# alshai/Big-BWT

Measured on NVIDIA B200. Metric: pfp_parse_throughput, higher is better.
Workload: dtype u8/u32/u64 integer

## Files before the change

### big-bwt_b200/csrc/pfp_phrase.cu

```cuda
#include "pfp_common.cuh"
#include "pfp_stages.cuh"
#include "pfp_fp.cuh"
#include <stdlib.h>

__device__ __forceinline__ void load_chunk(const TextView &tv, i64 s0, u64 len, u64 o, bool special,
                                           u32 x[4]) {
    const u32 nbv = (u32)((len - o) < 16 ? (len - o) : 16);
    if (!special) {
        const i64 loc = s0 + (i64)o - tv.pos0;
        const u8 *p = tv.T + loc;
        const u32 bs = (u32)((uintptr_t)p & 3);
        const u32 *p4 = reinterpret_cast<const u32 *>(p - bs);
        u32 W[5];
        if ((u64)loc + 20 <= tv.n_buf) {
#pragma unroll
            for (int j = 0; j < 5; j++) W[j] = __ldg(p4 + j);
        } else {
            const u32 need = bs + nbv;
#pragma unroll
            for (int j = 0; j < 5; j++) W[j] = (4u * j < need) ? __ldg(p4 + j) : 0u;
        }
#pragma unroll
        for (int j = 0; j < 4; j++) x[j] = __funnelshift_r(W[j], W[j + 1], 8 * bs);
    } else {
// ... 293 lines not shown
        const u32 slot = __shfl_sync(0xffffffffu, res, leader) & ~UID_CREATOR;
        const u32 lchk = __shfl_sync(0xffffffffu, chk, leader);
        if (j < P) {
            if (chk != lchk) atomicOr((unsigned long long *)&flags[0], PFP_ERRBIT_COLLISION);
            __stcs(uid + j, lead ? res : slot);
            if (weight) {
                const u32 c = weight[j];
                const u32 old = atomicAdd(&tab[slot].val, c);
                if (old + c < old) atomicOr((unsigned long long *)&flags[0], PFP_ERRBIT_LIMIT);
            }
        }
    }
}

constexpr int TC_T = 256;
constexpr int TC_I = 4;
constexpr int TC_TILE = TC_T * TC_I;

__device__ __forceinline__ void load_uids(const u32 *__restrict__ uid, u64 n, u64 j, u32 v[TC_I]) {
    if (j + TC_I <= n) {
        const uint4 a = __ldcs(reinterpret_cast<const uint4 *>(uid + j));
        v[0] = a.x; v[1] = a.y; v[2] = a.z; v[3] = a.w;
    } else {
#pragma unroll
        for (int i = 0; i < TC_I; i++) v[i] = j + i < n ? uid[j + i] : 0u;
    }
}

__global__ void __launch_bounds__(TC_T) table_creators_k(const u32 *__restrict__ uid, u64 n,
                                                         u32 *__restrict__ tile_count) {
    __shared__ u32 sm[9];
    u32 v[TC_I];
    load_uids(uid, n, (u64)blockIdx.x * TC_TILE + (u64)threadIdx.x * TC_I, v);
    u32 c = 0;
#pragma unroll
    for (int i = 0; i < TC_I; i++) c += v[i] >> 31;
    u32 total;
    block_excl_scan_256(c, &total, sm);
    if (threadIdx.x == 0) tile_count[blockIdx.x] = total;
}

__global__ void __launch_bounds__(TC_T, 6) table_compact_k(u32 *__restrict__ uid, u64 n,
                                                        const u32 *__restrict__ tile_base,
                                                        const DictSlot *__restrict__ tab,
                                                        const u32 *__restrict__ len_in,
                                                        const u64 *__restrict__ ends, i64 first_start, u32 w,
                                                        u32 *__restrict__ slot_of_word,
                                                        u32 *__restrict__ rep, u32 *__restrict__ count,
                                                        u32 *__restrict__ ulen, u32 *__restrict__ uwords,
                                                        i64 *__restrict__ ustart ,
                                                        u64 *__restrict__ flags) {
    __shared__ u32 sm[9];
    __shared__ u32 s_max;
    __shared__ unsigned long long s_sum;
    if (threadIdx.x == 0) { s_max = 0; s_sum = 0; }
    const u64 j0 = (u64)blockIdx.x * TC_TILE + (u64)threadIdx.x * TC_I;
    u32 v[TC_I];
    load_uids(uid, n, j0, v);
    u32 c = 0;
#pragma unroll
    for (int i = 0; i < TC_I; i++) c += v[i] >> 31;
    u32 cnt[TC_I], len[TC_I];
    i64 st[TC_I];
#pragma unroll
    for (int i = 0; i < TC_I; i++) {
        const u64 j = j0 + i;
        const bool cr = (v[i] & UID_CREATOR) != 0;
        cnt[i] = cr ? tab[v[i] & ~UID_CREATOR].val : 0u;
        if (len_in) {
            len[i] = cr ? len_in[j] : 0u;
            st[i] = 0;
        } else {
            st[i] = cr ? (j ? (i64)ends[j - 1] - (i64)w + 1 : first_start) : 0;
            len[i] = cr ? (u32)((i64)ends[j] - st[i] + 1) : 0u;
        }
    }
    u32 total;
    u32 u = block_excl_scan_256(c, &total, sm) + tile_base[blockIdx.x];
    u32 mx = 0;
    u64 sum = 0;
#pragma unroll
    for (int i = 0; i < TC_I; i++) {
        if (!(v[i] & UID_CREATOR)) continue;
        slot_of_word[u] = v[i] & ~UID_CREATOR;
        uid[j0 + i] = u | UID_CREATOR;
        rep[u] = (u32)(j0 + i); count[u] = cnt[i]; ulen[u] = len[i]; uwords[u] = (len[i] + 7) >> 3;
        if (ustart) ustart[u] = st[i];
        mx = max(mx, len[i]);
        sum += len[i];
        u++;
    }
    mx = __reduce_max_sync(0xffffffffu, mx);
#pragma unroll
    for (int o = 16; o > 0; o >>= 1) sum += __shfl_xor_sync(0xffffffffu, sum, o);
    if ((threadIdx.x & 31) == 0 && sum) { atomicMax(&s_max, mx); atomicAdd(&s_sum, (unsigned long long)sum); }
    __syncthreads();
    if (threadIdx.x == 0 && s_sum) {
        atomicMax((unsigned long long *)&flags[2], (unsigned long long)s_max);
        atomicAdd((unsigned long long *)&flags[3], s_sum);
    }
}

__global__ void word_of_slot_k(const u32 *__restrict__ slot_of_word, u64 d, const u64 *__restrict__ d_ptr,
                               u32 *__restrict__ word_of_slot) {
    const u64 u = (u64)blockIdx.x * blockDim.x + threadIdx.x;
    if (u < (d_ptr ? *d_ptr : d)) word_of_slot[slot_of_word[u]] = (u32)u;
}

__device__ __forceinline__ u32 word_of(u32 v, const u32 *__restrict__ word_of_slot) {
    return (v & UID_CREATOR) ? v & ~UID_CREATOR : word_of_slot[v];
}

__global__ void uid_words_k(u32 *__restrict__ uid, u64 n, const u32 *__restrict__ word_of_slot) {
    const u64 q = (u64)blockIdx.x * blockDim.x + threadIdx.x;
    const u64 j = 4 * q;
    if (j + 4 <= n) {
        uint4 v = __ldcs(reinterpret_cast<const uint4 *>(uid) + q);
        v.x = word_of(v.x, word_of_slot); v.y = word_of(v.y, word_of_slot);
        v.z = word_of(v.z, word_of_slot); v.w = word_of(v.w, word_of_slot);
        __stcs(reinterpret_cast<uint4 *>(uid) + q, v);
    } else {
        for (u64 i = j; i < n; i++) uid[i] = word_of(uid[i], word_of_slot);
    }
}

static int uid_words(pfpb200_ctx *ctx, DictArrays *D, u64 n, u64 d_max, const u64 *d_ptr) {
    if (n && d_max) {
        u32 *word_of_slot = nullptr;
        PFP_TRY(pfp_alloc_t(ctx, &word_of_slot, D->slots));
        word_of_slot_k<<<pfp_blocks(d_max, 256), 256, 0, ctx->stream>>>(D->slot_of_word, d_max, d_ptr, word_of_slot);
        PFP_LAUNCHED(ctx);
        uid_words_k<<<pfp_blocks((n + 3) / 4, 256), 256, 0, ctx->stream>>>(D->uid, n, word_of_slot);
        PFP_LAUNCHED(ctx);
        PFP_TRY(pfp_free_now(ctx, word_of_slot));
    }
    PFP_TRY(pfp_free_now(ctx, D->slot_of_word));
    D->slot_of_word = nullptr;
    return PFPB200_OK;
}

int pfp_uid_words(pfpb200_ctx *ctx, DictArrays *D, u64 n) {
    return D->slot_of_word ? uid_words(ctx, D, n, D->d, nullptr) : PFPB200_OK;
}

static int table_words(pfpb200_ctx *ctx, const PhraseFp *rec, u64 n, DictSlot *tab, u64 cap,
                       const u32 *weight, const u32 *len_in, const u64 *ends, i64 first_start, u32 w,
                       u32 *uid, const DictArrays &D) {
    table_init_k<<<pfp_blocks(cap, 256), 256, 0, ctx->stream>>>(tab, cap);
    PFP_LAUNCHED(ctx);
    PFP_CUDA(ctx, cudaMemsetAsync(&ctx->d_flags[1], 0, 3 * sizeof(u64), ctx->stream));
    if (n == 0) return PFPB200_OK;
    int per_sm = 0;
    PFP_CUDA(ctx, cudaOccupancyMaxActiveBlocksPerMultiprocessor(&per_sm, table_insert_k, TI_T, 0));
    const u64 want = (n + TI_T - 1) / TI_T;
    const u64 resident = (u64)ctx->sm_count * (per_sm > 0 ? per_sm : 1);
    table_insert_k<<<(u32)(want < resident ? want : resident), TI_T, 0, ctx->stream>>>(
        rec, n, tab, cap, weight, ctx->weak_fp, uid, ctx->d_flags);
    PFP_LAUNCHED(ctx);
    const u32 nt = pfp_blocks(n, TC_TILE);
    u32 *tile = nullptr;
    PFP_TRY(pfp_alloc_t(ctx, &tile, nt));
    table_creators_k<<<nt, TC_T, 0, ctx->stream>>>(uid, n, tile);
    PFP_LAUNCHED(ctx);
    PFP_TRY(pfp_exclusive_scan_u32(ctx, tile, tile, nt, reinterpret_cast<u32 *>(&ctx->d_flags[1])));
    table_compact_k<<<nt, TC_T, 0, ctx->stream>>>(uid, n, tile, tab, len_in, ends, first_start, w, D.slot_of_word,
                                                  D.rep, D.count, D.ulen, D.uwords, D.ustart, ctx->d_flags);
    PFP_LAUNCHED(ctx);
    PFP_TRY(pfp_free_now(ctx, tile));
    return PFPB200_OK;
}

__device__ __forceinline__ u64 phrase_word8(const TextView &tv, i64 s0, u64 len, u64 k, bool special) {
    const u64 o = 8 * k;
    const u32 nbv = (u32)((len - o) < 8 ? (len - o) : 8);
    u64 v = 0;
    if (!special) {
        const u8 *p = tv.T + (s0 + (i64)o - tv.pos0);
        const u32 bs = (u32)((uintptr_t)p & 7);
        const u64 *p8 = reinterpret_cast<const u64 *>(p - bs);
        const u64 lo = __ldg(p8);
        if (bs) {
            const u64 hi = (bs + nbv > 8) ? __ldg(p8 + 1) : 0ull;
            v = (lo >> (8 * bs)) | (hi << (64 - 8 * bs));
        } else v = lo;
    } else {
        for (u32 b = 0; b < nbv; b++) v |= (u64)tv_byte(tv, s0 + (i64)o + b) << (8 * b);
    }
    if (nbv < 8) v &= (1ull << (8 * nbv)) - 1ull;
    return v;
}

__global__ void __launch_bounds__(PH_T) pool_copy_span_k(TextView tv, const i64 *__restrict__ ustart,
                                                         const u32 *__restrict__ ulen,
                                                         const u64 *__restrict__ uoff, u64 d,
                                                         u64 *__restrict__ pool) {
    const u32 lane = threadIdx.x & 31;
    for (u64 u0 = ((u64)blockIdx.x * PH_WARPS + (threadIdx.x >> 5)) * 32; u0 < d; u0 += (u64)gridDim.x * PH_WARPS * 32) {
        const u64 u = u0 + lane;
        const bool have = u < d;
        const i64 s0 = have ? ustart[u] : 0;
        const u32 len = have ? ulen[u] : 0u;
        const u64 off = have ? uoff[u] : 0ull;
        const u64 base = __shfl_sync(0xffffffffu, off, 0);
        const u32 nw = (len + 7) >> 3;
        u32 rel = have ? (u32)(off - base) : 0xFFFFFFFFu;
        const u32 endrel = have ? rel + nw : 0u;
        u32 total = endrel;
#pragma unroll
        for (int o = 16; o > 0; o >>= 1) total = max(total, __shfl_xor_sync(0xffffffffu, total, o));
        const bool special = have && (s0 < 0 || s0 + (i64)len > tv.n_global);
        for (u32 k0 = 0; k0 < total; k0 += 32) {
            const u32 k = k0 + lane;
            u32 j = 0;
#pragma unroll
            for (int step = 16; step > 0; step >>= 1) {
                const u32 t = __shfl_sync(0xffffffffu, rel, (j + step) & 31);
                if (j + step < 32 && t <= k) j += step;
            }
            const u32 rj = __shfl_sync(0xffffffffu, rel, j);
            const u32 lj = __shfl_sync(0xffffffffu, len, j);
            const i64 sj = __shfl_sync(0xffffffffu, s0, j);
            const int spj = __shfl_sync(0xffffffffu, (int)special, j);
            if (k < total) pool[base + k] = phrase_word8(tv, sj, lj, k - rj, spj != 0);
        }
    }
}

__global__ void __launch_bounds__(PH_T) verify_phrases_k(TextView tv, const u64 *__restrict__ ends,
                                                         i64 first_start, u32 w, u64 P,
                                                         const u32 *__restrict__ uid,
                                                         const u32 *__restrict__ ulen,
                                                         const u64 *__restrict__ uoff,
                                                         const u64 *__restrict__ pool,
                                                         u64 *__restrict__ flags) {
    const u32 lane = threadIdx.x & 31;
    for (u64 j = (u64)blockIdx.x * PH_WARPS + (threadIdx.x >> 5); j < P; j += (u64)gridDim.x * PH_WARPS) {
        const i64 e = (i64)ends[j];
        const i64 s0 = (j == 0) ? first_start : (i64)ends[j - 1] - (i64)w + 1;
        const u64 len = (u64)(e - s0 + 1);
        const u32 u = uid[j];
        bool bad = len != (u64)ulen[u];
        if (!bad) {
            const bool special = (s0 < 0) || (e >= tv.n_global);
            const u64 *src = pool + uoff[u];
            const u64 nw = (len + 7) >> 3;
            for (u64 k = lane; k < nw; k += 32) bad |= phrase_word8(tv, s0, len, k, special) != src[k];
        }
        if (__any_sync(0xffffffffu, bad) && lane == 0)
            atomicOr((unsigned long long *)&flags[0], PFP_ERRBIT_COLLISION);
    }
}

__global__ void __launch_bounds__(PH_T) verify_entries_k(u64 n, const u32 *__restrict__ uid_of_entry,
                                                         const u32 *__restrict__ rep,
                                                         const u32 *__restrict__ len_in,
                                                         const u64 *__restrict__ in_off,
                                                         const u64 *__restrict__ pool,
                                                         u64 *__restrict__ flags) {
    const u32 lane = threadIdx.x & 31;
    for (u64 i = (u64)blockIdx.x * PH_WARPS + (threadIdx.x >> 5); i < n; i += (u64)gridDim.x * PH_WARPS) {
        const u32 r = rep[uid_of_entry[i]];
        if (r == (u32)i) continue;
        bool bad = len_in[i] != len_in[r];
        if (!bad) {
            const u64 *a = pool + in_off[i], *b = pool + in_off[r];
            const u64 nw = ((u64)len_in[i] + 7) >> 3;
            for (u64 k = lane; k < nw; k += 32) bad |= a[k] != b[k];
        }
        if (__any_sync(0xffffffffu, bad) && lane == 0)
            atomicOr((unsigned long long *)&flags[0], PFP_ERRBIT_COLLISION);
    }
}

int pfp_hash_list(pfpb200_ctx *ctx, const TextView &tv, const PhraseArrays &ph, i64 first_start, u32 w,
                  const u32 *long_list, const u32 *long_count, u64 max_count) {
    u64 want = (max_count + PH_WARPS - 1) / PH_WARPS;
// ... 8 lines not shown
}

int pfp_records_range(pfpb200_ctx *ctx, const TextView &tv, const PhraseArrays &ph, u64 j0, u64 P, u32 w) {
    if (j0 >= P) return PFPB200_OK;
    phrase_records_k<<<pfp_blocks(P - j0, 256), 256, 0, ctx->stream>>>(tv, ph.ends, j0, P, w, ph.last, ph.sai);
    PFP_LAUNCHED(ctx);
    return PFPB200_OK;
}

int pfp_hash_stage(pfpb200_ctx *ctx, const TextView &tv, const PhraseArrays &ph, u64 P,
                   i64 first_start, u32 w) {
    u32 *long_list = nullptr, *long_count = nullptr;
    const u64 cap = P + 8;
    PFP_TRY(pfp_alloc_t(ctx, &long_list, (size_t)cap));
    PFP_TRY(pfp_alloc_t(ctx, &long_count, 1));
    PFP_CUDA(ctx, cudaMemsetAsync(long_count, 0, sizeof(u32), ctx->stream));
    phrase_records_k<<<pfp_blocks(P, 256), 256, 0, ctx->stream>>>(tv, ph.ends, 0, P, w, ph.last, ph.sai);
    PFP_LAUNCHED(ctx);
    u64 want = (P + PH_PER_BLOCK - 1) / PH_PER_BLOCK;
    u64 maxb = (u64)ctx->sm_count * 32;
    u32 nb = (u32)(want < maxb ? want : maxb);
    if (nb == 0) nb = 1;
    phrase_hash_k<<<nb, PH_T, 0, ctx->stream>>>(tv, ph, P, first_start, w, ctx->d_keys, long_list, long_count,
                                                (u32)cap, ctx->d_flags);
    PFP_LAUNCHED(ctx);
    PFP_TRY(pfp_hash_list(ctx, tv, ph, first_start, w, long_list, long_count, cap));
    PFP_TRY(pfp_free_now(ctx, long_list));
    PFP_TRY(pfp_free_now(ctx, long_count));
    return PFPB200_OK;
}

int pfp_dedup_stage(pfpb200_ctx *ctx, const PhraseArrays &ph, u64 P, i64 first_start, u32 w, DictArrays *D) {
    if (P >= 0x7FFFFFFEull) return pfp_fail(ctx, PFPB200_E_LIMIT, "more than 2^31-2 phrases in one shard");
    DictSlot *tab = nullptr;
    u64 cap = 0, d = 0;
    PFP_TRY(pfp_alloc_t(ctx, &D->uid, P));
    for (int attempt = 0;; attempt++) {
        double want = (double)P * 1.5;
        if (attempt == 0 && ctx->dedup_ratio > 0.0) {
            double guess = ctx->dedup_ratio * (double)P * 2.0;
            if (guess < want) want = guess;
        }
        cap = (u64)want + 1024;
        if (cap >= 0x7FFFFFFFull) cap = 0x7FFFFFFEull;
        const u64 wcap = cap < P ? cap : P;
        PFP_TRY(pfp_alloc_t(ctx, &tab, cap));
        PFP_TRY(pfp_alloc_t(ctx, &D->slot_of_word, wcap));
        PFP_TRY(pfp_alloc_t(ctx, &D->rep, wcap));
        PFP_TRY(pfp_alloc_t(ctx, &D->count, wcap));
        PFP_TRY(pfp_alloc_t(ctx, &D->ulen, wcap));
        PFP_TRY(pfp_alloc_t(ctx, &D->uwords, wcap));
        PFP_TRY(pfp_alloc_t(ctx, &D->ustart, wcap));
        PFP_TRY(table_words(ctx, ph.rec, P, tab, cap, nullptr, nullptr, ph.ends, first_start, w, D->uid, *D));
        PFP_CUDA(ctx, cudaMemcpyAsync(ctx->h_flags, ctx->d_flags, 4 * sizeof(u64), cudaMemcpyDeviceToHost,
                                      ctx->stream));
        PFP_CUDA(ctx, cudaStreamSynchronize(ctx->stream));
        if (ctx->h_flags[0] & PFP_ERRBIT_LIMIT)
            return pfp_fail(ctx, PFPB200_E_LIMIT, "a phrase is longer than 2^32-1 bytes");
        d = ctx->h_flags[1];
        const bool full = (ctx->h_flags[0] & PFP_ERRBIT_TABLE_FULL) != 0 || (double)d > 0.85 * (double)cap;
        if (!full) break;
        if (attempt > 0) return pfp_fail(ctx, PFPB200_E_INTERNAL, "dictionary table overflow");
        void *fr[] = {tab, D->slot_of_word, D->rep, D->count, D->ulen, D->uwords, D->ustart};
        for (void *q : fr) PFP_TRY(pfp_free_now(ctx, q));
        ctx->dedup_ratio = 0.0;
        const u64 keep = ctx->h_flags[0] & ~(PFP_ERRBIT_TABLE_FULL | PFP_ERRBIT_COLLISION);
        PFP_CUDA(ctx, cudaMemcpyAsync(&ctx->d_flags[0], &keep, sizeof(u64), cudaMemcpyHostToDevice, ctx->stream));
        PFP_CUDA(ctx, cudaStreamSynchronize(ctx->stream));
    }
    D->slots = cap;
    ctx->dedup_ratio = (double)d / (double)P;
    if (d > 0x7FFFFFFEull)
        return pfp_fail(ctx, PFPB200_E_LIMIT, "%llu distinct words exceed the limit 2^31-2",
                        (unsigned long long)d);
    D->d = d;
    D->max_len = (u32)ctx->h_flags[2];
    D->sum_len = ctx->h_flags[3];
    PFP_TRY(pfp_free_now(ctx, tab));
    return PFPB200_OK;
}

int pfp_pool_stage(pfpb200_ctx *ctx, const TextView &tv, DictArrays *D) {
    u64 d = D->d;
    PFP_TRY(pfp_alloc_t(ctx, &D->uoff, d));
    PFP_TRY(pfp_exclusive_scan_u32_u64(ctx, D->uwords, D->uoff, d, &ctx->d_flags[1]));
    PFP_CUDA(ctx, cudaMemcpyAsync(ctx->h_flags, ctx->d_flags, 4 * sizeof(u64), cudaMemcpyDeviceToHost,
                                  ctx->stream));
    PFP_CUDA(ctx, cudaStreamSynchronize(ctx->stream));
    if (ctx->h_flags[0] & PFP_ERRBIT_COLLISION)
        return pfp_fail(ctx, PFPB200_E_COLLISION, "fingerprint collision between different phrases");
    D->pool_words = ctx->h_flags[1];
    D->max_len = (u32)ctx->h_flags[2];
    D->sum_len = ctx->h_flags[3];
    PFP_TRY(pfp_alloc_t(ctx, &D->pool, (size_t)D->pool_words));
    u64 want = (d + 32ull * PH_WARPS - 1) / (32ull * PH_WARPS);
    u64 maxb = (u64)ctx->sm_count * 32;
    pool_copy_span_k<<<(u32)(want < maxb ? (want ? want : 1) : maxb), PH_T, 0, ctx->stream>>>(
        tv, D->ustart, D->ulen, D->uoff, d, D->pool);
    PFP_LAUNCHED(ctx);
    return PFPB200_OK;
}

int pfp_merge_verify(pfpb200_ctx *ctx, u64 n, const u32 *uid_of_entry, const u32 *rep, const u32 *len_in,
                     const u32 *uwords_in, const u64 *pool) {
    if (n == 0) return PFPB200_OK;
    u64 *in_off = nullptr;
    PFP_TRY(pfp_alloc_t(ctx, &in_off, n));
    PFP_TRY(pfp_exclusive_scan_u32_u64(ctx, uwords_in, in_off, n, nullptr));
    u64 want = (n + PH_WARPS - 1) / PH_WARPS;
    u64 maxb = (u64)ctx->sm_count * 32;
    verify_entries_k<<<(u32)(want < maxb ? want : maxb), PH_T, 0, ctx->stream>>>(n, uid_of_entry, rep, len_in, in_off, pool,
                                                                                ctx->d_flags);
    PFP_LAUNCHED(ctx);
    PFP_CUDA(ctx, cudaMemcpyAsync(ctx->h_flags, ctx->d_flags, sizeof(u64), cudaMemcpyDeviceToHost, ctx->stream));
    PFP_CUDA(ctx, cudaStreamSynchronize(ctx->stream));
    PFP_TRY(pfp_free_now(ctx, in_off));
    if (ctx->h_flags[0] & PFP_ERRBIT_COLLISION)
        return pfp_fail(ctx, PFPB200_E_COLLISION, "two different words share a fingerprint (found by the verify pass)");
    return PFPB200_OK;
}

int pfp_verify_stage(pfpb200_ctx *ctx, const TextView &tv, const u64 *ends, i64 first_start, u32 w, u64 P,
                     const DictArrays &D) {
    if (P == 0) return PFPB200_OK;
    u64 want = (P + PH_WARPS - 1) / PH_WARPS;
    u64 maxb = (u64)ctx->sm_count * 32;
    verify_phrases_k<<<(u32)(want < maxb ? want : maxb), PH_T, 0, ctx->stream>>>(
        tv, ends, first_start, w, P, D.uid, D.ulen, D.uoff, D.pool, ctx->d_flags);
    PFP_LAUNCHED(ctx);
    return PFPB200_OK;
}

__global__ void merge_recs_k(const u64 *__restrict__ fpa, const u64 *__restrict__ fpb, u64 n,
                             PhraseFp *__restrict__ rec) {
    u64 i = (u64)blockIdx.x * blockDim.x + threadIdx.x;
    if (i < n) store_rec(rec, i, fpa[i], fpb[i]);
}

__global__ void merge_words_k(const u32 *__restrict__ rep, const u32 *__restrict__ uwords_in,
                              const u64 *__restrict__ in_off, const u64 *__restrict__ d_ptr,
                              u32 *__restrict__ uwords, u64 *__restrict__ uoff) {
    u64 u = (u64)blockIdx.x * blockDim.x + threadIdx.x;
    if (u >= *d_ptr) return;
    const u32 r = rep[u];
    uwords[u] = uwords_in[r];
    uoff[u] = in_off[r];
}

__global__ void gather_word_fp_k(const u32 *__restrict__ rep, const PhraseFp *__restrict__ rec,
// ... 75 lines not shown
```

### big-bwt_b200/csrc/pfp_rank.cu

```cuda
#include "pfp_common.cuh"
#include "pfp_stages.cuh"

__device__ __forceinline__ u64 bswap64(u64 v) {
    u32 lo = (u32)v, hi = (u32)(v >> 32);
    return ((u64)__byte_perm(lo, 0, 0x0123) << 32) | (u64)__byte_perm(hi, 0, 0x0123);
}

__device__ __forceinline__ u64 word_key(const u64 *__restrict__ pool, const u64 *__restrict__ uoff,
                                        const u32 *__restrict__ uwords, u32 u, u32 r) {
    return (r < uwords[u]) ? bswap64(__ldg(pool + uoff[u] + r)) : 0ull;
}

struct AlphaMap {
    u32 bits;
    u32 chars;
    u32 depth0;
    u32 pad;
    u8 lut[256];
};

constexpr u32 ALPHA_PROBE_WORDS = 3;

__global__ void alpha_presence_k(const u64 *__restrict__ pool, const u64 *__restrict__ uoff,
                                 const u32 *__restrict__ ulen, u64 d, u32 *__restrict__ gmask) {
// ... 17 lines not shown
        for (int q = 0; q < 8; q++) {
            u32 x = __reduce_or_sync(__activemask(), m[q]);
            if ((threadIdx.x & 31) == (__ffs(__activemask()) - 1) && x) atomicOr(&sm[q], x);
        }
    }
    __syncthreads();
    if (threadIdx.x < 8 && sm[threadIdx.x]) atomicOr(&gmask[threadIdx.x], sm[threadIdx.x]);
}

__global__ void alpha_build_k(u32 *__restrict__ gmask, AlphaMap *am, int from_scan) {
    if (threadIdx.x != 0 || blockIdx.x != 0) return;
    if (from_scan) {
        gmask[0] |= 1u << PFP_DOLLAR;
        gmask[2] |= (1u << ('A' & 31)) | (1u << ('C' & 31)) | (1u << ('G' & 31)) | (1u << ('T' & 31));
    }
    u32 sigma = 0;
    for (int q = 0; q < 8; q++) sigma += __popc(gmask[q]);
    u32 bits = 3;
    while ((1u << bits) < sigma + 1) bits++;
    if (bits > 4) {
        am->bits = 8; am->chars = 8; am->depth0 = 1;
        for (int c = 0; c < 256; c++) am->lut[c] = (u8)c;
    } else {
        am->bits = bits; am->chars = 64 / bits; am->depth0 = (64 / bits) / 8;
        u32 code = 0;
        for (int c = 0; c < 256; c++) {
            bool present = (gmask[c >> 5] >> (c & 31)) & 1u;
            if (present) code++;
            am->lut[c] = (u8)(present ? code : 0);
        }
    }
    am->pad = 0;
}

__global__ void rank_keys0_k(const u64 *__restrict__ pool, const u64 *__restrict__ uoff,
                             const u32 *__restrict__ ulen, const u32 *__restrict__ count, u64 d,
                             const AlphaMap *__restrict__ am, u64 *__restrict__ keys, u32 *__restrict__ vals,
                             WordMeta *__restrict__ meta) {
    __shared__ u8 lut[256];
    __shared__ u32 s_bits, s_chars;
    lut[threadIdx.x & 255] = am->lut[threadIdx.x & 255];
    if (threadIdx.x == 0) { s_bits = am->bits; s_chars = am->chars; }
    __syncthreads();
    u64 u = (u64)blockIdx.x * blockDim.x + threadIdx.x;
    if (u >= d) return;
    const u32 bits = s_bits, chars = s_chars, len = ulen[u];
    const u64 off = uoff[u];
    {
        WordMeta wm;
        wm.off = off; wm.len = len; wm.count = count[u];
        meta[u] = wm;
    }
    const u32 nc = len < chars ? len : chars;
    u64 key = 0;
    u64 v = 0;
    for (u32 i = 0; i < nc; i++) {
        if ((i & 7) == 0) v = __ldg(pool + off + (i >> 3));
        u32 c = (u32)(v >> (8 * (i & 7))) & 255u;
        key |= (u64)lut[c] << (64 - bits * (i + 1));
    }
    keys[u] = key;
    vals[u] = (u32)u;
}

__global__ void rank_heads0_k(const u64 *__restrict__ ks, u64 d, const AlphaMap *__restrict__ am, u32 begin_bit,
                              u8 *__restrict__ head, u32 *__restrict__ depth) {
    u64 i = (u64)blockIdx.x * blockDim.x + threadIdx.x;
    if (i >= d) return;
    head[i] = (i == 0 || (ks[i] >> begin_bit) != (ks[i - 1] >> begin_bit)) ? 1 : 0;
    const u32 chars = (64u - begin_bit) / am->bits;
    const u32 d0 = chars / 8u;
    depth[i] = d0 < am->depth0 ? d0 : am->depth0;
}

constexpr u32 LOCAL_MAX = 2048;
constexpr u32 WARP_MAX = 32;

__global__ void groups_compact_k(const u8 *__restrict__ head, const u32 *__restrict__ hscan, u64 d,
                                 const u32 *__restrict__ nheads, u32 *__restrict__ hp,
                                 u32 *__restrict__ gid) {
    u64 i = (u64)blockIdx.x * blockDim.x + threadIdx.x;
    if (i >= d) return;
    u32 g = hscan[i] + head[i] - 1;
    gid[i] = g;
    if (head[i]) hp[g] = (u32)i;
    if (i == 0) hp[*nheads] = (u32)d;
}

__global__ void rank_active_k(u8 *__restrict__ head, const u32 *__restrict__ gid,
                              const u32 *__restrict__ hp, u64 d, u8 *__restrict__ act,
                              u8 *__restrict__ gh) {
    u64 i = (u64)blockIdx.x * blockDim.x + threadIdx.x;
    if (i >= d) return;
    u32 g = gid[i];
    bool big = (hp[g + 1] - hp[g]) > LOCAL_MAX;
    act[i] = big ? 1 : 0;
    gh[i] = (big && head[i]) ? 1 : 0;
    if (!big) head[i] = 1;
}

__global__ void rank_compact_k(const u8 *__restrict__ act, const u8 *__restrict__ gh,
                               const u32 *__restrict__ ascan, const u32 *__restrict__ gscan,
                               const u32 *__restrict__ ord, const u32 *__restrict__ gid,
                               const u32 *__restrict__ hp, const u32 *__restrict__ depth, u64 d,
                               const u64 *pool, const u64 *uoff, const u32 *uwords,
                               u32 *__restrict__ apos, u64 *__restrict__ keys, u32 *__restrict__ vals,
                               u32 *__restrict__ gid_of_u) {
    u64 i = (u64)blockIdx.x * blockDim.x + threadIdx.x;
    if (i >= d || !act[i]) return;
    u32 j = ascan[i];
    u32 u = ord[i];
// ... 935 lines not shown
        rank_gidkeys_k<<<nbm, TB, 0, ctx->stream>>>(vs, gid_of_u, m, g_in);
        PFP_LAUNCHED(ctx);
        int bits = 1;
        while (bits < 32 && (1ull << bits) < ng) bits++;
        u64 *gs = nullptr;
        u32 *vs2 = nullptr;
        PFP_TRY(pfp_radix_sort_pairs(ctx, g_in, vs, ks, v_other, m, 0, bits, &gs, &vs2));
        PFP_CUDA(ctx, cudaMemcpyAsync(depth2, depth, d * sizeof(u32), cudaMemcpyDeviceToDevice, ctx->stream));
        rank_writeback_k<<<nbm, TB, 0, ctx->stream>>>(apos, gs, vs2, m, gid, hp, depth, D.pool, D.uoff,
                                                      D.uwords, ord, head, depth2);
        PFP_LAUNCHED(ctx);
        u32 *tdp = depth; depth = depth2; depth2 = tdp;
    }
    *rounds = r;
    *order = ord;
    void *to_free[] = {k0, k1, v0, v1, depth, depth2, hscan, hp, gid, head, am, amask, act, gh, ascan,
                       gscan, apos, gid_of_u};
    for (void *q : to_free) PFP_TRY(pfp_free_now(ctx, q));
    return PFPB200_OK;
}

__device__ __forceinline__ void out_span(const u64 *pool, u64 off, u32 len, u32 strip_w, u32 *skip,
                                         u32 *outlen) {
    *skip = 0;
    *outlen = len;
    if (strip_w) {
        u32 l = len - strip_w;
        if ((u8)(pool[off] & 0xFF) == PFP_DOLLAR) { *skip = 1; l -= 1; }
        *outlen = l;
    }
}

__global__ void dict_layout_k(const u32 *__restrict__ ord, u64 d, const DictArrays D, u32 strip_w,
                              u32 *__restrict__ rank_of_uid, u32 *__restrict__ occ,
                              u32 *__restrict__ dl) {
    u64 i = (u64)blockIdx.x * blockDim.x + threadIdx.x;
    if (i >= d) return;
    u32 u = ord[i];
    rank_of_uid[u] = (u32)i + 1;
    const uint4 mv = __ldg(reinterpret_cast<const uint4 *>(D.meta + u));
    occ[i] = mv.w;
    u32 skip, outlen;
    out_span(D.pool, ((u64)mv.y << 32) | mv.x, mv.z, strip_w, &skip, &outlen);
    dl[i] = outlen + 1;
}

__global__ void rank_of_slot_k(const u32 *__restrict__ slot_of_word, const u32 *__restrict__ count,
                               const u32 *__restrict__ rank_of_uid, u64 d, u32 *__restrict__ rank_of_slot) {
    u64 u = (u64)blockIdx.x * blockDim.x + threadIdx.x;
    if (u < d && count[u] > 1) rank_of_slot[slot_of_word[u]] = rank_of_uid[u];
}

constexpr int DC_T = 256;
constexpr int DC_GROUP = 8;

__global__ void __launch_bounds__(DC_T) dict_copy_k(const u32 *__restrict__ ord,
                                                    const u64 *__restrict__ doff, u64 d,
                                                    const DictArrays D, u32 strip_w, u64 total,
                                                    u8 *__restrict__ dict) {
    const u32 li = threadIdx.x & (DC_GROUP - 1);
    if (blockIdx.x == 0 && threadIdx.x == 0) dict[total] = (u8)PFP_END_OF_DICT;
    for (u64 i = (u64)blockIdx.x * (DC_T / DC_GROUP) + (threadIdx.x / DC_GROUP); i < d;
         i += (u64)gridDim.x * (DC_T / DC_GROUP)) {
        const u32 u = ord[i];
        u32 skip, outlen;
        const uint4 mv = __ldg(reinterpret_cast<const uint4 *>(D.meta + u));
        const u64 off = ((u64)mv.y << 32) | mv.x;
        out_span(D.pool, off, mv.z, strip_w, &skip, &outlen);
        const u64 *src64 = D.pool + off;
        const u8 *src = reinterpret_cast<const u8 *>(src64) + skip;
        u8 *dst = dict + doff[i];
        u32 head = (u32)((8 - ((uintptr_t)dst & 7)) & 7);
        if (head > outlen) head = outlen;
        if (li < head) dst[li] = src[li];
        const u32 nbody = (outlen - head) >> 3;
        u64 *dst64 = reinterpret_cast<u64 *>(dst + head);
        for (u32 k = li; k < nbody; k += DC_GROUP) {
            u32 so = skip + head + 8 * k;
            u32 sh = (so & 7) * 8;
            u64 w0 = __ldg(src64 + (so >> 3));
            u64 v = w0;
            if (sh) v = (w0 >> sh) | (__ldg(src64 + (so >> 3) + 1) << (64 - sh));
            dst64[k] = v;
        }
        const u32 done = head + 8 * nbody;
        if (li < outlen - done) dst[done + li] = src[done + li];
        if (li == DC_GROUP - 1) dst[outlen] = (u8)PFP_END_OF_WORD;
    }
}

__global__ void remap_k(const u32 *__restrict__ uid, const u32 *__restrict__ rank_of_uid, u64 P,
                        u32 *__restrict__ parse, const u32 *__restrict__ rank_of_slot);

int pfp_dict_stage(pfpb200_ctx *ctx, const DictArrays &D, const u32 *order, u32 strip_w, u8 **dict,
                   u64 *dict_bytes, u32 **occ, u32 **rank_of_uid, const u32 *remap_uid, u64 remap_n,
                   u32 *remap_out) {
    const int TB = 256;
    const u64 d = D.d;
    u32 *dl = nullptr;
    u64 *doff = nullptr;
    PFP_TRY(pfp_alloc_t(ctx, occ, d, true));
    PFP_TRY(pfp_alloc_t(ctx, rank_of_uid, d));
    PFP_TRY(pfp_alloc_t(ctx, &dl, d));
    PFP_TRY(pfp_alloc_t(ctx, &doff, d));
    const bool side_remap = remap_uid && remap_out && remap_n;
    u32 *rank_of_slot = nullptr;
    if (side_remap && D.slot_of_word) PFP_TRY(pfp_alloc_t(ctx, &rank_of_slot, D.slots));
    dict_layout_k<<<pfp_blocks(d, TB), TB, 0, ctx->stream>>>(order, d, D, strip_w, *rank_of_uid, *occ, dl);
    PFP_LAUNCHED(ctx);
    if (side_remap) {
        PFP_CUDA(ctx, cudaEventRecord(ctx->ev_aux0, ctx->stream));
        PFP_CUDA(ctx, cudaStreamWaitEvent(ctx->aux_stream, ctx->ev_aux0, 0));
        if (rank_of_slot) {
            rank_of_slot_k<<<pfp_blocks(d, TB), TB, 0, ctx->aux_stream>>>(D.slot_of_word, D.count, *rank_of_uid, d,
                                                                          rank_of_slot);
            PFP_LAUNCHED(ctx);
        }
        remap_k<<<pfp_blocks((remap_n + 3) / 4, 256), 256, 0, ctx->aux_stream>>>(remap_uid, *rank_of_uid, remap_n,
                                                                                 remap_out, rank_of_slot);
        PFP_LAUNCHED(ctx);
        PFP_CUDA(ctx, cudaEventRecord(ctx->ev_aux1, ctx->aux_stream));
    }
    PFP_TRY(pfp_exclusive_scan_u32_u64(ctx, dl, doff, d, &ctx->d_flags[1]));
    PFP_CUDA(ctx, cudaMemcpyAsync(&ctx->h_flags[1], &ctx->d_flags[1], sizeof(u64),
                                  cudaMemcpyDeviceToHost, ctx->stream));
    PFP_CUDA(ctx, cudaStreamSynchronize(ctx->stream));
    u64 total = ctx->h_flags[1];
    *dict_bytes = total + 1;
    PFP_TRY(pfp_alloc_t(ctx, dict, (size_t)(total + 1), true));
    u64 want = (d + (DC_T / DC_GROUP) - 1) / (DC_T / DC_GROUP);
    u64 maxb = (u64)ctx->sm_count * 32;
    u32 nb = (u32)(want < maxb ? want : maxb);
    if (nb == 0) nb = 1;
    dict_copy_k<<<nb, DC_T, 0, ctx->stream>>>(order, doff, d, D, strip_w, total, *dict);
    PFP_LAUNCHED(ctx);
    if (side_remap) PFP_CUDA(ctx, cudaStreamWaitEvent(ctx->stream, ctx->ev_aux1, 0));
    PFP_TRY(pfp_free_now(ctx, rank_of_slot));
    PFP_TRY(pfp_free_now(ctx, dl));
    PFP_TRY(pfp_free_now(ctx, doff));
    return PFPB200_OK;
}

__device__ __forceinline__ u32 rank_of(u32 v, const u32 *__restrict__ rank_of_uid, const u32 *__restrict__ rank_of_slot) {
    if (rank_of_slot && !(v & UID_CREATOR)) return __ldg(rank_of_slot + v);
    return __ldg(rank_of_uid + (v & ~UID_CREATOR));
}

__global__ void remap_k(const u32 *__restrict__ uid, const u32 *__restrict__ rank_of_uid, u64 P,
                        u32 *__restrict__ parse, const u32 *__restrict__ rank_of_slot) {
    const u64 q = (u64)blockIdx.x * blockDim.x + threadIdx.x;
    const u64 j = 4 * q;
    if (j + 4 <= P && (((uintptr_t)uid | (uintptr_t)parse) & 15) == 0) {
        const uint4 v = __ldcs(reinterpret_cast<const uint4 *>(uid) + q);
        uint4 r;
        r.x = rank_of(v.x, rank_of_uid, rank_of_slot); r.y = rank_of(v.y, rank_of_uid, rank_of_slot);
        r.z = rank_of(v.z, rank_of_uid, rank_of_slot); r.w = rank_of(v.w, rank_of_uid, rank_of_slot);
        reinterpret_cast<uint4 *>(parse)[q] = r;
    } else {
        for (u64 i = j; i < P && i < j + 4; i++) parse[i] = rank_of(uid[i], rank_of_uid, rank_of_slot);
    }
}

int pfp_remap_stage(pfpb200_ctx *ctx, const u32 *uid, const u32 *rank_of_uid, u64 P, u32 *parse) {
    remap_k<<<pfp_blocks((P + 3) / 4, 256), 256, 0, ctx->stream>>>(uid, rank_of_uid, P, parse, nullptr);
    PFP_LAUNCHED(ctx);
    return PFPB200_OK;
}

struct Splitters { u64 s[PFPB200_MAX_RANKS]; u32 n; };

__global__ void first_keys_k(const u64 *__restrict__ pool, const u64 *__restrict__ uoff,
                             const u32 *__restrict__ uwords, u64 d, u64 *__restrict__ keys) {
    u64 u = (u64)blockIdx.x * blockDim.x + threadIdx.x;
    if (u < d) keys[u] = word_key(pool, uoff, uwords, (u32)u, 0);
}

__global__ void route_dest_k(const u64 *__restrict__ pool, const u64 *__restrict__ uoff,
                             const u32 *__restrict__ uwords, u64 d, Splitters sp,
                             u64 *__restrict__ keys, u32 *__restrict__ vals,
                             unsigned long long *__restrict__ cnt ) {
    __shared__ unsigned long long sc[2 * PFPB200_MAX_RANKS];
    for (int i = threadIdx.x; i < 2 * PFPB200_MAX_RANKS; i += blockDim.x) sc[i] = 0;
    __syncthreads();
    u64 u = (u64)blockIdx.x * blockDim.x + threadIdx.x;
    if (u < d) {
        u64 k = word_key(pool, uoff, uwords, (u32)u, 0);
        u32 dest = 0;
// ... 327 lines not shown
```

Baseline: 532.0.

## Vectorize pool and dict copies, drop host syncs for pool size and dict total

Pool word totals are now computed during table compaction, so the pool stage no longer needs a scan-total readback and host sync. The dict stage skips its sync when strip_w is zero and takes the total from sum_len+d. The pool copy kernel stages per-warp phrase metadata in shared memory and writes four 64-bit words per thread with 16-byte stores. The dict copy kernel uses 16-byte aligned stores with a templated group size chosen from average phrase length. The rank key build also unrolls its byte loads. The risks are extra shared-memory pressure, subtle boundary handling in the new copy paths, and reliance on sum_len being exact.

Result: no change. 537.2 (median of 6 runs) (+1.0%).

```diff
diff --git a/big-bwt_b200/csrc/pfp_phrase.cu b/big-bwt_b200/csrc/pfp_phrase.cu
--- a/big-bwt_b200/csrc/pfp_phrase.cu
+++ b/big-bwt_b200/csrc/pfp_phrase.cu
@@ -369,8 +369,8 @@
                                                         u64 *__restrict__ flags) {
     __shared__ u32 sm[9];
     __shared__ u32 s_max;
-    __shared__ unsigned long long s_sum;
-    if (threadIdx.x == 0) { s_max = 0; s_sum = 0; }
+    __shared__ unsigned long long s_sum, s_words;
+    if (threadIdx.x == 0) { s_max = 0; s_sum = 0; s_words = 0; }
     const u64 j0 = (u64)blockIdx.x * TC_TILE + (u64)threadIdx.x * TC_I;
     u32 v[TC_I];
     load_uids(uid, n, j0, v);
@@ -395,26 +395,36 @@
     u32 total;
     u32 u = block_excl_scan_256(c, &total, sm) + tile_base[blockIdx.x];
     u32 mx = 0;
-    u64 sum = 0;
+    u64 sum = 0, words = 0;
 #pragma unroll
     for (int i = 0; i < TC_I; i++) {
         if (!(v[i] & UID_CREATOR)) continue;
+        const u32 nw = (len[i] + 7) >> 3;
         slot_of_word[u] = v[i] & ~UID_CREATOR;
         uid[j0 + i] = u | UID_CREATOR;
-        rep[u] = (u32)(j0 + i); count[u] = cnt[i]; ulen[u] = len[i]; uwords[u] = (len[i] + 7) >> 3;
+        rep[u] = (u32)(j0 + i); count[u] = cnt[i]; ulen[u] = len[i]; uwords[u] = nw;
         if (ustart) ustart[u] = st[i];
         mx = max(mx, len[i]);
         sum += len[i];
+        words += nw;
         u++;
     }
     mx = __reduce_max_sync(0xffffffffu, mx);
 #pragma unroll
-    for (int o = 16; o > 0; o >>= 1) sum += __shfl_xor_sync(0xffffffffu, sum, o);
-    if ((threadIdx.x & 31) == 0 && sum) { atomicMax(&s_max, mx); atomicAdd(&s_sum, (unsigned long long)sum); }
+    for (int o = 16; o > 0; o >>= 1) {
+        sum += __shfl_xor_sync(0xffffffffu, sum, o);
+        words += __shfl_xor_sync(0xffffffffu, words, o);
+    }
+    if ((threadIdx.x & 31) == 0 && sum) {
+        atomicMax(&s_max, mx);
+        atomicAdd(&s_sum, (unsigned long long)sum);
+        atomicAdd(&s_words, (unsigned long long)words);
+    }
     __syncthreads();
     if (threadIdx.x == 0 && s_sum) {
         atomicMax((unsigned long long *)&flags[2], (unsigned long long)s_max);
         atomicAdd((unsigned long long *)&flags[3], s_sum);
+        atomicAdd((unsigned long long *)&flags[4], s_words);
     }
 }
 
@@ -465,7 +475,7 @@
                        u32 *uid, const DictArrays &D) {
     table_init_k<<<pfp_blocks(cap, 256), 256, 0, ctx->stream>>>(tab, cap);
     PFP_LAUNCHED(ctx);
-    PFP_CUDA(ctx, cudaMemsetAsync(&ctx->d_flags[1], 0, 3 * sizeof(u64), ctx->stream));
+    PFP_CUDA(ctx, cudaMemsetAsync(&ctx->d_flags[1], 0, 4 * sizeof(u64), ctx->stream));
     if (n == 0) return PFPB200_OK;
     int per_sm = 0;
     PFP_CUDA(ctx, cudaOccupancyMaxActiveBlocksPerMultiprocessor(&per_sm, table_insert_k, TI_T, 0));
@@ -507,38 +517,76 @@
     return v;
 }
 
-__global__ void __launch_bounds__(PH_T) pool_copy_span_k(TextView tv, const i64 *__restrict__ ustart,
-                                                         const u32 *__restrict__ ulen,
-                                                         const u64 *__restrict__ uoff, u64 d,
-                                                         u64 *__restrict__ pool) {
-    const u32 lane = threadIdx.x & 31;
-    for (u64 u0 = ((u64)blockIdx.x * PH_WARPS + (threadIdx.x >> 5)) * 32; u0 < d; u0 += (u64)gridDim.x * PH_WARPS * 32) {
+constexpr u32 PC_SLOTS = 4;
+
+__global__ void __launch_bounds__(PH_T, 6) pool_copy_span_k(TextView tv, const i64 *__restrict__ ustart,
+                                                            const u32 *__restrict__ ulen,
+                                                            const u64 *__restrict__ uoff, u64 d,
+                                                            u64 *__restrict__ pool) {
+    __shared__ u32 s_rel[PH_WARPS][33];
+    __shared__ u32 s_len[PH_WARPS][32];
+    __shared__ i64 s_st[PH_WARPS][32];
+    const u32 lane = threadIdx.x & 31, wi = threadIdx.x >> 5;
+    u32 *rel = s_rel[wi], *lens = s_len[wi];
+    i64 *sts = s_st[wi];
+    for (u64 u0 = ((u64)blockIdx.x * PH_WARPS + wi) * 32; u0 < d; u0 += (u64)gridDim.x * PH_WARPS * 32) {
         const u64 u = u0 + lane;
         const bool have = u < d;
+        const u64 off = have ? uoff[u] : 0ull;
+        const u32 len = have ? ulen[u] : 0u;
         const i64 s0 = have ? ustart[u] : 0;
-        const u32 len = have ? ulen[u] : 0u;
-        const u64 off = have ? uoff[u] : 0ull;
         const u64 base = __shfl_sync(0xffffffffu, off, 0);
-        const u32 nw = (len + 7) >> 3;
-        u32 rel = have ? (u32)(off - base) : 0xFFFFFFFFu;
-        const u32 endrel = have ? rel + nw : 0u;
-        u32 total = endrel;
-#pragma unroll
-        for (int o = 16; o > 0; o >>= 1) total = max(total, __shfl_xor_sync(0xffffffffu, total, o));
-        const bool special = have && (s0 < 0 || s0 + (i64)len > tv.n_global);
-        for (u32 k0 = 0; k0 < total; k0 += 32) {
-            const u32 k = k0 + lane;
+        const u64 abase = base & ~(u64)(PC_SLOTS - 1);
+        const u32 lo = (u32)(base - abase);
+        const u32 hi = __reduce_max_sync(0xffffffffu, have ? (u32)(off - abase) + ((len + 7) >> 3) : 0u);
+        __syncwarp();
+        rel[lane] = have ? (u32)(off - abase) : 0xFFFFFFFFu;
+        lens[lane] = len;
+        sts[lane] = s0;
+        if (lane == 0) rel[32] = 0xFFFFFFFFu;
+        __syncwarp();
+        for (u32 k = PC_SLOTS * lane; k < hi; k += 32 * PC_SLOTS) {
+            const u32 kf = k > lo ? k : lo;
             u32 j = 0;
 #pragma unroll
-            for (int step = 16; step > 0; step >>= 1) {
-                const u32 t = __shfl_sync(0xffffffffu, rel, (j + step) & 31);
-                if (j + step < 32 && t <= k) j += step;
+            for (int step = 16; step > 0; step >>= 1)
+                if (rel[j + step] <= kf) j += step;
+            const u32 rj = rel[j], lj = lens[j];
+            const i64 sj = sts[j];
+            const u32 rn = rel[j + 1];
+            u64 *dst = pool + abase + k;
+            if (k >= lo && k + PC_SLOTS <= (rn < hi ? rn : hi) && sj >= 0 && sj + (i64)lj <= tv.n_global) {
+                const u32 ob = 8 * (k - rj);
+                const u32 nb = lj - ob < 8 * PC_SLOTS ? lj - ob : 8 * PC_SLOTS;
+                const u8 *p = tv.T + (sj + (i64)ob - tv.pos0);
+                const u32 bs = (u32)((uintptr_t)p & 7);
+                const u64 *p8 = reinterpret_cast<const u64 *>(p - bs);
+                u64 w[PC_SLOTS + 1];
+#pragma unroll
+                for (u32 q = 0; q <= PC_SLOTS; q++) w[q] = 8 * q < bs + nb ? __ldg(p8 + q) : 0ull;
+                if (bs) {
+#pragma unroll
+                    for (u32 q = 0; q < PC_SLOTS; q++) w[q] = (w[q] >> (8 * bs)) | (w[q + 1] << (64 - 8 * bs));
+                }
+                if (nb < 8 * PC_SLOTS) w[PC_SLOTS - 1] &= (1ull << (8 * (nb - 8 * (PC_SLOTS - 1)))) - 1ull;
+                reinterpret_cast<ulonglong2 *>(dst)[0] = make_ulonglong2(w[0], w[1]);
+                reinterpret_cast<ulonglong2 *>(dst)[1] = make_ulonglong2(w[2], w[3]);
+            } else {
+                u64 v[PC_SLOTS];
+#pragma unroll
+                for (u32 q = 0; q < PC_SLOTS; q++) {
+                    const u32 kk = k + q;
+                    v[q] = 0;
+                    if (kk < lo || kk >= hi) continue;
+                    while (rel[j + 1] <= kk) j++;
+                    const i64 s = sts[j];
+                    const u32 l = lens[j];
+                    v[q] = phrase_word8(tv, s, l, kk - rel[j], s < 0 || s + (i64)l > tv.n_global);
+                }
+#pragma unroll
+                for (u32 q = 0; q < PC_SLOTS; q++)
+                    if (k + q >= lo && k + q < hi) dst[q] = v[q];
             }
-            const u32 rj = __shfl_sync(0xffffffffu, rel, j);
-            const u32 lj = __shfl_sync(0xffffffffu, len, j);
-            const i64 sj = __shfl_sync(0xffffffffu, s0, j);
-            const int spj = __shfl_sync(0xffffffffu, (int)special, j);
-            if (k < total) pool[base + k] = phrase_word8(tv, sj, lj, k - rj, spj != 0);
         }
     }
 }
@@ -653,7 +701,7 @@
         PFP_TRY(pfp_alloc_t(ctx, &D->uwords, wcap));
         PFP_TRY(pfp_alloc_t(ctx, &D->ustart, wcap));
         PFP_TRY(table_words(ctx, ph.rec, P, tab, cap, nullptr, nullptr, ph.ends, first_start, w, D->uid, *D));
-        PFP_CUDA(ctx, cudaMemcpyAsync(ctx->h_flags, ctx->d_flags, 4 * sizeof(u64), cudaMemcpyDeviceToHost,
+        PFP_CUDA(ctx, cudaMemcpyAsync(ctx->h_flags, ctx->d_flags, 5 * sizeof(u64), cudaMemcpyDeviceToHost,
                                       ctx->stream));
         PFP_CUDA(ctx, cudaStreamSynchronize(ctx->stream));
         if (ctx->h_flags[0] & PFP_ERRBIT_LIMIT)
@@ -674,28 +722,23 @@
     if (d > 0x7FFFFFFEull)
         return pfp_fail(ctx, PFPB200_E_LIMIT, "%llu distinct words exceed the limit 2^31-2",
                         (unsigned long long)d);
+    if (ctx->h_flags[0] & PFP_ERRBIT_COLLISION)
+        return pfp_fail(ctx, PFPB200_E_COLLISION, "fingerprint collision between different phrases");
     D->d = d;
     D->max_len = (u32)ctx->h_flags[2];
     D->sum_len = ctx->h_flags[3];
+    D->pool_words = ctx->h_flags[4];
     PFP_TRY(pfp_free_now(ctx, tab));
     return PFPB200_OK;
 }
 
 int pfp_pool_stage(pfpb200_ctx *ctx, const TextView &tv, DictArrays *D) {
-    u64 d = D->d;
+    const u64 d = D->d;
     PFP_TRY(pfp_alloc_t(ctx, &D->uoff, d));
-    PFP_TRY(pfp_exclusive_scan_u32_u64(ctx, D->uwords, D->uoff, d, &ctx->d_flags[1]));
-    PFP_CUDA(ctx, cudaMemcpyAsync(ctx->h_flags, ctx->d_flags, 4 * sizeof(u64), cudaMemcpyDeviceToHost,
-                                  ctx->stream));
-    PFP_CUDA(ctx, cudaStreamSynchronize(ctx->stream));
-    if (ctx->h_flags[0] & PFP_ERRBIT_COLLISION)
-        return pfp_fail(ctx, PFPB200_E_COLLISION, "fingerprint collision between different phrases");
-    D->pool_words = ctx->h_flags[1];
-    D->max_len = (u32)ctx->h_flags[2];
-    D->sum_len = ctx->h_flags[3];
+    PFP_TRY(pfp_exclusive_scan_u32_u64(ctx, D->uwords, D->uoff, d, nullptr));
     PFP_TRY(pfp_alloc_t(ctx, &D->pool, (size_t)D->pool_words));
-    u64 want = (d + 32ull * PH_WARPS - 1) / (32ull * PH_WARPS);
-    u64 maxb = (u64)ctx->sm_count * 32;
+    const u64 want = (d + 32ull * PH_WARPS - 1) / (32ull * PH_WARPS);
+    const u64 maxb = (u64)ctx->sm_count * 32;
     pool_copy_span_k<<<(u32)(want < maxb ? (want ? want : 1) : maxb), PH_T, 0, ctx->stream>>>(
         tv, D->ustart, D->ulen, D->uoff, d, D->pool);
     PFP_LAUNCHED(ctx);
diff --git a/big-bwt_b200/csrc/pfp_rank.cu b/big-bwt_b200/csrc/pfp_rank.cu
--- a/big-bwt_b200/csrc/pfp_rank.cu
+++ b/big-bwt_b200/csrc/pfp_rank.cu
@@ -93,11 +93,14 @@
         meta[u] = wm;
     }
     const u32 nc = len < chars ? len : chars;
+    u64 v[3];
+#pragma unroll
+    for (u32 q = 0; q < 3; q++) v[q] = 8 * q < nc ? __ldg(pool + off + q) : 0ull;
     u64 key = 0;
-    u64 v = 0;
-    for (u32 i = 0; i < nc; i++) {
-        if ((i & 7) == 0) v = __ldg(pool + off + (i >> 3));
-        u32 c = (u32)(v >> (8 * (i & 7))) & 255u;
+#pragma unroll
+    for (u32 i = 0; i < 24; i++) {
+        if (i >= nc) break;
+        const u32 c = (u32)(v[i >> 3] >> (8 * (i & 7))) & 255u;
         key |= (u64)lut[c] << (64 - bits * (i + 1));
     }
     keys[u] = key;
@@ -1139,16 +1142,19 @@
 }
 
 constexpr int DC_T = 256;
-constexpr int DC_GROUP = 8;
-
+
+__device__ __forceinline__ u64 funnel8(u64 lo, u64 hi, u32 sh) {
+    return sh ? (lo >> sh) | (hi << (64 - sh)) : lo;
+}
+
+template <u32 G>
 __global__ void __launch_bounds__(DC_T) dict_copy_k(const u32 *__restrict__ ord,
                                                     const u64 *__restrict__ doff, u64 d,
                                                     const DictArrays D, u32 strip_w, u64 total,
                                                     u8 *__restrict__ dict) {
-    const u32 li = threadIdx.x & (DC_GROUP - 1);
+    const u32 li = threadIdx.x & (G - 1);
     if (blockIdx.x == 0 && threadIdx.x == 0) dict[total] = (u8)PFP_END_OF_DICT;
-    for (u64 i = (u64)blockIdx.x * (DC_T / DC_GROUP) + (threadIdx.x / DC_GROUP); i < d;
-         i += (u64)gridDim.x * (DC_T / DC_GROUP)) {
+    for (u64 i = (u64)blockIdx.x * (DC_T / G) + (threadIdx.x / G); i < d; i += (u64)gridDim.x * (DC_T / G)) {
         const u32 u = ord[i];
         u32 skip, outlen;
         const uint4 mv = __ldg(reinterpret_cast<const uint4 *>(D.meta + u));
@@ -1157,22 +1163,31 @@
         const u64 *src64 = D.pool + off;
         const u8 *src = reinterpret_cast<const u8 *>(src64) + skip;
         u8 *dst = dict + doff[i];
-        u32 head = (u32)((8 - ((uintptr_t)dst & 7)) & 7);
+        u32 head = (u32)((16 - ((uintptr_t)dst & 15)) & 15);
         if (head > outlen) head = outlen;
-        if (li < head) dst[li] = src[li];
-        const u32 nbody = (outlen - head) >> 3;
-        u64 *dst64 = reinterpret_cast<u64 *>(dst + head);
-        for (u32 k = li; k < nbody; k += DC_GROUP) {
-            u32 so = skip + head + 8 * k;
-            u32 sh = (so & 7) * 8;
-            u64 w0 = __ldg(src64 + (so >> 3));
-            u64 v = w0;
-            if (sh) v = (w0 >> sh) | (__ldg(src64 + (so >> 3) + 1) << (64 - sh));
-            dst64[k] = v;
-        }
-        const u32 done = head + 8 * nbody;
-        if (li < outlen - done) dst[done + li] = src[done + li];
-        if (li == DC_GROUP - 1) dst[outlen] = (u8)PFP_END_OF_WORD;
+        const u32 nbody = (outlen - head) >> 4;
+        const u32 done = head + 16 * nbody;
+        const u32 sb = skip + head;
+        const u32 sh = (sb & 7) * 8;
+        const u64 *s8 = src64 + (sb >> 3);
+        ulonglong2 *dst16 = reinterpret_cast<ulonglong2 *>(dst + head);
+        for (u32 c = li; c < nbody; c += 2 * G) {
+            const u32 c2 = c + G;
+            const bool two = c2 < nbody;
+            const u64 a0 = __ldg(s8 + 2 * c), a1 = __ldg(s8 + 2 * c + 1);
+            const u64 a2 = sh ? __ldg(s8 + 2 * c + 2) : 0ull;
+            u64 b0 = 0, b1 = 0, b2 = 0;
+            if (two) {
+                b0 = __ldg(s8 + 2 * c2);
+                b1 = __ldg(s8 + 2 * c2 + 1);
+                if (sh) b2 = __ldg(s8 + 2 * c2 + 2);
+            }
+            dst16[c] = make_ulonglong2(funnel8(a0, a1, sh), funnel8(a1, a2, sh));
+            if (two) dst16[c2] = make_ulonglong2(funnel8(b0, b1, sh), funnel8(b1, b2, sh));
+        }
+        for (u32 b = li; b < head; b += G) dst[b] = src[b];
+        for (u32 b = done + li; b < outlen; b += G) dst[b] = src[b];
+        if (li == G - 1) dst[outlen] = (u8)PFP_END_OF_WORD;
     }
 }
 
@@ -1208,18 +1223,26 @@
         PFP_LAUNCHED(ctx);
         PFP_CUDA(ctx, cudaEventRecord(ctx->ev_aux1, ctx->aux_stream));
     }
-    PFP_TRY(pfp_exclusive_scan_u32_u64(ctx, dl, doff, d, &ctx->d_flags[1]));
-    PFP_CUDA(ctx, cudaMemcpyAsync(&ctx->h_flags[1], &ctx->d_flags[1], sizeof(u64),
-                                  cudaMemcpyDeviceToHost, ctx->stream));
-    PFP_CUDA(ctx, cudaStreamSynchronize(ctx->stream));
-    u64 total = ctx->h_flags[1];
+    u64 total = D.sum_len + d;
+    if (strip_w) {
+        PFP_TRY(pfp_exclusive_scan_u32_u64(ctx, dl, doff, d, &ctx->d_flags[1]));
+        PFP_CUDA(ctx, cudaMemcpyAsync(&ctx->h_flags[1], &ctx->d_flags[1], sizeof(u64),
+                                      cudaMemcpyDeviceToHost, ctx->stream));
+        PFP_CUDA(ctx, cudaStreamSynchronize(ctx->stream));
+        total = ctx->h_flags[1];
+    } else {
+        PFP_TRY(pfp_exclusive_scan_u32_u64(ctx, dl, doff, d, nullptr));
+    }
     *dict_bytes = total + 1;
     PFP_TRY(pfp_alloc_t(ctx, dict, (size_t)(total + 1), true));
-    u64 want = (d + (DC_T / DC_GROUP) - 1) / (DC_T / DC_GROUP);
-    u64 maxb = (u64)ctx->sm_count * 32;
+    const bool wide = d && D.sum_len / d > 128;
+    const u64 G = wide ? 8 : 4;
+    const u64 want = (d + (DC_T / G) - 1) / (DC_T / G);
+    const u64 maxb = (u64)ctx->sm_count * 32;
     u32 nb = (u32)(want < maxb ? want : maxb);
     if (nb == 0) nb = 1;
-    dict_copy_k<<<nb, DC_T, 0, ctx->stream>>>(order, doff, d, D, strip_w, total, *dict);
+    if (wide) dict_copy_k<8><<<nb, DC_T, 0, ctx->stream>>>(order, doff, d, D, strip_w, total, *dict);
+    else dict_copy_k<4><<<nb, DC_T, 0, ctx->stream>>>(order, doff, d, D, strip_w, total, *dict);
     PFP_LAUNCHED(ctx);
     if (side_remap) PFP_CUDA(ctx, cudaStreamWaitEvent(ctx->stream, ctx->ev_aux1, 0));
     PFP_TRY(pfp_free_now(ctx, rank_of_slot));
```
